# moskewcz/boda

Hardware: AMD Instinct MI355X
Metric: effective TFLOP/s (2*M*N*K / time), whole job (higher is better)
Workload: dtype f32

## Files before the change

__graft_entry__.py:

```python
from __future__ import annotations
import os
import sys

ROOT = os.path.dirname(os.path.abspath(__file__))
if ROOT not in sys.path:
    sys.path.insert(0, ROOT)


def build() -> None:
    from boda_amd import build as b
    so = b.build()
    assert os.path.exists(so)
    import boda_amd.rtc as rtc
    from boda_amd import gen_data
    from boda_amd.op import read_ops
    assert rtc._lib.bodahip_abi_version() == 1
    rtc.compile_offline(gen_data.SRC, use_cache=True)
    n = 0
    gold = os.path.join(ROOT, "tests", "golden", "ops")
    for fn in ("sgemm-ops-full.txt", "sgemm-ops-debug-half.txt", "conv-ops-1-5-20-nin-alex-gn.txt", "conv-ops-debug.txt", "conv-ops-debug-tmp.txt",
               "bck-conv-ops.txt", "bck-ops.txt", "bck-pipe-ops.txt", "bck-fuse-ops.txt", "bck-graph-ops.txt", "bck-shards-ops.txt", "resnet-ops.txt", "fwd-deps-ops.txt", "sgd-ops.txt", "bn-ops.txt", "bconv-fb-ops.txt", "bconv-bf16-ops.txt"):
        if not os.path.exists(os.path.join(gold, fn)):
            continue
        for op in read_ops(os.path.join(gold, fn)):
            rtc.prebuild(op); n += 1
    import bench
    from boda_amd.cnn_op import OpTune, add_codegen_annotations
    from boda_amd import conv_pipe
    rtc.compile_offline(conv_pipe.FWD_SRC, use_cache=True)
    for op in bench.alexnet_b256_ops() + bench.nin_ops() + bench.net_conv_ops("googlenet_conv", 64) + bench.net_conv_ops("resnet-50", 64):
        rtc.prebuild(op); n += 1
    for op in bench.net_conv_ops("googlenet_conv", 2) + bench.net_conv_ops("resnet-50", 2) + bench.alexnet_b256_ops(2) + bench.nin_ops(3):
        rtc.prebuild(op); n += 1
    for op in bench.alexnet_b256_ops() + bench.nin_ops() + bench.sgemm_full_ops() + bench.net_conv_ops("googlenet_conv", 64) + bench.net_conv_ops("resnet-50", 64):
        rtc.prebuild(add_codegen_annotations(op, OpTune(hip_dtype="bf16"))); n += 1
    from boda_amd import nhwc
    rtc.compile_offline(nhwc.XPOSE_SRC, use_cache=True)
    for op in bench.net_conv_ops("googlenet_conv", 64) + bench.net_conv_ops("resnet-50", 64) + bench.net_conv_ops("googlenet_conv", 2) + bench.net_conv_ops("resnet-50", 2):
        for out in ("", "f32"):
            rtc.prebuild(add_codegen_annotations(op, OpTune(hip_dtype="bf16", hip_layout="nhwc", hip_out=out))); n += 1
    for net in ("googlenet_conv", "resnet-50"):
        for out in ("", "f32"):
            el = [x for x in (add_codegen_annotations(op, OpTune(hip_dtype="bf16", hip_layout="nhwc", hip_out=out)) for op in bench.net_conv_ops(net, 64)) if nhwc.multi_eligible(x)]
            m = nhwc.annotate_multi(el); rtc.prebuild(m); n += 1
            for t in ("64x128x64x2x2x2", "128x128x64x2x2x2", "32x128x64x1x4x2", "32x128x64x1x4x2x1x32x2", "128x64x32x2x2x2x1x32x4", "64x64x32x2x2x2x1x32x3"):
                rtc.prebuild(m, tile=t); n += 1
    from boda_amd.conv_pipe import ConvPipeFwd, DryRtc
    seen = set()
    resnet_small = lambda batch: conv_pipe.resnet50(batch, 64)
    for make, batches, kw in ((conv_pipe.googlenet_conv, (64, 1, 3), {}), (conv_pipe.nin_imagenet, (256, 128, 2), {}), (conv_pipe.alexnet_ng_conv, (256, 2), {}),
                              (conv_pipe.resnet50, (64,), {}), (conv_pipe.resnet50, (64,), {"fuse_residual": False}), (resnet_small, (2,), {}), (resnet_small, (2,), {"fuse_residual": False})):
        for batch in batches:
            dry = DryRtc(); ConvPipeFwd(dry, OpTune(hip_dtype="bf16", hip_layout="nhwc"), **kw).init(make(batch))
            for fi in dry.infos:
                if fi.op is not None and fi.op.has_func_name() and fi.op.get_func_name().startswith("hip_conv_nhwc") and "_xpose_" not in fi.op.get_func_name() and fi.op.to_str() not in seen:
                    seen.add(fi.op.to_str()); rtc.prebuild(fi.op); n += 1
    for batch in (256, 128):
        dry = DryRtc(); ConvPipeFwd(dry).init(conv_pipe.nin_imagenet(batch))
        for fi in dry.infos:
            if fi.op is not None and fi.op.has_func_name() and fi.op.get_func_name() == "hip_conv_k1_chain" and fi.op.to_str() not in seen:
                seen.add(fi.op.to_str()); rtc.prebuild(fi.op); n += 1
    dry = DryRtc(); ConvPipeFwd(dry).init(resnet_small(2))
    for fi in dry.infos:
        if fi.op is not None and fi.op.has_func_name() and fi.op.get_func_name() in ("hip_conv", "hip_chan_affine", "hip_reduce", "hip_zero_if_non_pos") and fi.op.to_str() not in seen:
            seen.add(fi.op.to_str()); rtc.prebuild(fi.op); n += 1
    _recompile_with_the_wheels_hiprtc()
    b.build_adapter()
    from oracle import boda_oracle, ref_cucl
    boda_oracle.build()
    n_ref = ref_cucl.build()
    print(f"oracle/_ref/cucl: {n_ref} reference kernels compiled" if n_ref else "oracle/_ref/cucl: no Boda checkout here, prebuilt files (if any) left alone")
    print(f"build ok: {so}; {n} ops pre-specialised into {os.path.join(ROOT, 'boda_amd', '_kcache')}")


def _fp32_conv_ops():
    import bench
    ops = bench.alexnet_b256_ops() + bench.nin_ops() + bench.nin_ops(128) + bench.net_conv_ops("googlenet_conv", 64) + bench.net_conv_ops("resnet-50", 64)
    return ops + bench.net_conv_ops("googlenet_conv", 2) + bench.net_conv_ops("resnet-50", 2) + bench.alexnet_b256_ops(2) + bench.nin_ops(3)


def _recompile_with_the_wheels_hiprtc() -> None:
    import subprocess
    code = ("import torch, os, sys; sys.path.insert(0, %r); os.environ['BODAHIP_CACHE_REFRESH'] = 'bodahip_conv_big'\n"
            "import __graft_entry__ as g, boda_amd.rtc as rtc\n"
            "n = 0\n"
            "for op in g._fp32_conv_ops():\n"
            "    if rtc.explain_plan(op).startswith('bodahip_conv_big_f32'): rtc.prebuild(op); n += 1\n"
            "print(n)" % ROOT)
    r = subprocess.run([sys.executable, "-c", code], capture_output=True, text=True, timeout=1800)
    if r.returncode != 0:
        print("build: second pass (the wheel's hiprtc for the staging-wave convolution kernels) skipped: " + (r.stderr.strip().splitlines() or ["?"])[-1])
    else:
        print(f"build: {r.stdout.strip().splitlines()[-1]} staging-wave convolution plans recompiled by the PyTorch wheel's hiprtc")


def smoke() -> None:
    import numpy as np
    from boda_amd.cnn_op import OpTune, add_codegen_annotations
    from boda_amd.op import parse_op
    from boda_amd.ops_prof import OpsBackend, profile_rcg_call
    from boda_amd.rtc import make_rtc
    from oracle import boda_oracle as bo
    rtc = make_rtc("(be=hip)", 0)
    rtc.init()
    be = OpsBackend(rtc)
    sg = parse_op("(str_vals=(type=sgemm),nda_vals=(a=(dims=(K=192,M=256)),b=(dims=(K=192,N=320)),c=(dims=(M=256,N=320))))")
    outs, prc = profile_rcg_call(be, add_codegen_annotations(sg, OpTune()), 5, include_ins=True)
    assert np.array_equal(outs["c"], bo.sgemm(outs["a"], outs["b"])), "smoke: sgemm mismatch vs oracle"
    cv = parse_op("(str_vals=(type=Convolution),nda_vals=(biases=(dims=(out_chan=64)),filts=(dims=(out_chan=64,in_chan=32,y=5,x=5)),"
                  "in=(dims=(img=5,chan=32,y=14,x=14)),in_pad=(tn=none,dims=(y=2,x=2)),kern_sz=(tn=none,dims=(y=5,x=5)),"
                  "out=(dims=(img=5,chan=64,y=14,x=14)),out_chans=(tn=uint32_t,v=64),stride=(tn=none,dims=(y=1,x=1))))")
    outs, prc2 = profile_rcg_call(be, add_codegen_annotations(cv, OpTune()), 5, include_ins=True)
    want = bo.conv_fwd(outs["in"], outs["filts"], outs["biases"], (1, 1), (2, 2), True)
    assert np.array_equal(outs["out"], want), "smoke: conv mismatch vs oracle"
    t_s, t_c = "64x64x16x2x2x4x1x32x2x3", "64x128x16x2x2x2x1x32x2x2"
    outs, prc3 = profile_rcg_call(be, add_codegen_annotations(sg, OpTune(hip_tile=t_s)), 5, include_ins=True, tile=t_s)
    assert prc3.launch["kernel"] == "bodahip_sgemm_big_f32" and np.array_equal(outs["c"], bo.sgemm(outs["a"], outs["b"])), "smoke: staging-wave sgemm mismatch vs oracle"
    outs, prc4 = profile_rcg_call(be, add_codegen_annotations(cv, OpTune(hip_tile=t_c)), 5, include_ins=True, tile=t_c)
    assert prc4.launch["kernel"] == "bodahip_conv_big_f32" and np.array_equal(outs["out"], want), "smoke: staging-wave conv mismatch vs oracle"
    print(f"smoke ok on {rtc.get_plat_tag()}: sgemm {prc.rt_secs*1e6:.1f} us [{prc.launch['cfg']}] / [{prc3.launch['cfg']}], conv {prc2.rt_secs*1e6:.1f} us [{prc2.launch['cfg']}] / [{prc4.launch['cfg']}]")
    rtc.close()


if __name__ == "__main__":
    build()
    if len(sys.argv) > 1 and sys.argv[1] == "smoke":
        smoke()
```

boda_amd/csrc/kernels/sgemm_big_f32.hip:

```cpp

#ifndef __HIPCC_RTC__
#include <hip/hip_runtime.h>
#endif

typedef float f32x16 __attribute__((ext_vector_type(16)));
typedef float f32x4 __attribute__((ext_vector_type(4)));
typedef unsigned u32x2 __attribute__((ext_vector_type(2)));
#ifndef GROUP_I
#define GROUP_I 8
#endif
#ifndef BKS
#define BKS 8
#endif
#ifndef PF
#define PF 2
#endif
#ifndef TBI
#define TBI 256
#endif
#ifndef TBJ
#define TBJ 256
#endif
#ifndef WI
#define WI 2
#endif
#ifndef WJ
#define WJ 4
#endif
#ifndef MINW
#define MINW 1
#endif
#ifndef MULPRIO
#define MULPRIO 1
#endif
#ifndef STGPRIO
#define STGPRIO 0
#endif
#ifndef NSTG
#define NSTG 4
#endif

struct gemm_args_t {
  float const *I; float const *J; float *D; float const *bias;
  int Mi, Nj, K;
  int ldI, ldJ, ldD;
  int C, H, W, OH, OW;
  int tiles_i, tiles_j;
  int splitk, kt_per;
  float *ws; long ws_slab;
  unsigned I_bytes, J_bytes;
  unsigned D_bytes;
  int out_ctot, out_coff;
  int const *ktab; int ktab_n;
  long bsI, bsJ, bsD;
};

namespace {
constexpr int kNMW = WI * WJ;
static_assert(kNMW == 8 || kNMW == 4, "eight (or four) multiplying waves");
constexpr int kTI = TBI / (WI * 32), kTJ = TBJ / (WJ * 32);
static_assert(TBI % (WI * 32) == 0 && TBJ % (WJ * 32) == 0 && (kTI == 4 || kTI == 2 || kTI == 1) && (kTJ == 2 || kTJ == 1), "wave tile: 4 | 2 | 1 row blocks x 2 | 1 column blocks");
constexpr int kLDI = TBI + 4, kLDJ = TBJ + 4;
constexpr int kImgI = BKS * kLDI, kImgJ = BKS * kLDJ, kImg2 = kImgI + kImgJ;
constexpr int kNLI = BKS * (TBI / 4) / 256, kNLJ = BKS * (TBJ / 4) / 256;
static_assert((BKS * (TBI / 4)) % 256 == 0 && (BKS * (TBJ / 4)) % 256 == 0, "whole float4 units per staging thread");
constexpr int kKK = BKS / 2;
constexpr int kU = (NSTG == 3) ? 3 * PF : ((PF > NSTG) ? PF : NSTG);
constexpr int kD = NSTG - 1;
static_assert(NSTG == 3 || NSTG == 4, "NSTG: 3 | 4");
constexpr int kOOB = (int)0x80000000;
static_assert(BKS % 4 == 0 && (PF == 2 || PF == 4), "BKS % 4 == 0, PF: 2 | 4");
typedef __amdgpu_buffer_rsrc_t rsrc_t;
__device__ __forceinline__ rsrc_t make_rsrc(float const *p, unsigned bytes) { return __builtin_amdgcn_make_buffer_rsrc((void *)p, 0, (int)bytes, 0x00020000); }
__device__ __forceinline__ f32x4 bload4(rsrc_t r, int voff, int soff) { return __builtin_bit_cast(f32x4, __builtin_amdgcn_raw_buffer_load_b128(r, voff, soff, 0)); }
}

#if (TBI / (WI * 32)) == 4
typedef f32x4 avec_t;
#elif (TBI / (WI * 32)) == 2
typedef float2 avec_t;
#else
typedef float avec_t;
#endif
#if (TBJ / (WJ * 32)) == 2
typedef float2 bvec_t;
#else
typedef float bvec_t;
#endif
namespace {
__device__ __forceinline__ float vget(f32x4 const &v, int i) { return v[i]; }
__device__ __forceinline__ float vget(float2 const &v, int i) { return i ? v.y : v.x; }
__device__ __forceinline__ float vget(float const &v, int) { return v; }
}

extern "C" __global__ __launch_bounds__((kNMW + 4) * 64, MINW) void KNAME(gemm_args_t const p) {
  __shared__ __attribute__((aligned(16))) float sm[NSTG * kImg2];
  int const lane = threadIdx.x & 63;
  int const wave = __builtin_amdgcn_readfirstlane(threadIdx.x >> 6);
  bool const stager = wave >= kNMW;

  int tile_i, tile_j;
  {
    int const bid = blockIdx.x, nb = p.tiles_i * p.tiles_j;
    int const q = nb >> 3, rr = nb & 7, xcd = bid & 7, idx = bid >> 3;
    int const nid = ((xcd < rr) ? xcd * (q + 1) : rr * (q + 1) + (xcd - rr) * q) + idx;
    int const group_sz = GROUP_I * p.tiles_j, gid = nid / group_sz, first_i = gid * GROUP_I;
    int const gsz = min(p.tiles_i - first_i, GROUP_I), in_g = nid - gid * group_sz;
    tile_i = first_i + in_g % gsz; tile_j = in_g / gsz;
  }
  int const i0 = tile_i * TBI, j0 = tile_j * TBJ;
  int const nkt = (p.K + BKS - 1) / BKS;
  int const nkt_pad = (nkt + kU - 1) / kU * kU;

  if (stager) {
#if STGPRIO
    __builtin_amdgcn_s_setprio(STGPRIO);
#endif
    int const tid = threadIdx.x - kNMW * 64;
    rsrc_t const rI = make_rsrc(p.I, p.I_bytes), rJ = make_rsrc(p.J, p.J_bytes);
    int goffI[kNLI], goffJ[kNLJ], loffI[kNLI], loffJ[kNLJ], krowI[kNLI], krowJ[kNLJ];
#pragma unroll
    for (int n = 0; n < kNLI; ++n) {
      int const c = tid + n * 256, kr = c / (TBI / 4), x = 4 * (c % (TBI / 4));
      krowI[n] = kr; loffI[n] = kr * kLDI + x;
      goffI[n] = (i0 + x < p.Mi) ? ((kr * p.ldI + i0 + x) * 4) : kOOB;
    }
#pragma unroll
    for (int n = 0; n < kNLJ; ++n) {
      int const c = tid + n * 256, kr = c / (TBJ / 4), x = 4 * (c % (TBJ / 4));
      krowJ[n] = kr; loffJ[n] = kImgI + kr * kLDJ + x;
      goffJ[n] = (j0 + x < p.Nj) ? ((kr * p.ldJ + j0 + x) * 4) : kOOB;
    }
    auto gloadI = [&](int n, int kt) -> f32x4 { return bload4(rI, (kt * BKS + krowI[n] < p.K) ? goffI[n] : kOOB, min(kt, nkt - 1) * (BKS * 4) * p.ldI); };
    auto gloadJ = [&](int n, int kt) -> f32x4 { return bload4(rJ, (kt * BKS + krowJ[n] < p.K) ? goffJ[n] : kOOB, min(kt, nkt - 1) * (BKS * 4) * p.ldJ); };
    auto lstoreI = [&](int n, int stage, f32x4 const &v) { *reinterpret_cast<f32x4 *>(sm + stage * kImg2 + loffI[n]) = v; };
    auto lstoreJ = [&](int n, int stage, f32x4 const &v) { *reinterpret_cast<f32x4 *>(sm + stage * kImg2 + loffJ[n]) = v; };
    f32x4 ringI[PF][kNLI], ringJ[PF][kNLJ];
#pragma unroll
    for (int u = 0; u < PF; ++u) {
#pragma unroll
      for (int n = 0; n < kNLI; ++n) ringI[u][n] = gloadI(n, u);
#pragma unroll
      for (int n = 0; n < kNLJ; ++n) ringJ[u][n] = gloadJ(n, u);
    }
#pragma unroll
    for (int t = 0; t < kD; ++t) {
#pragma unroll
      for (int n = 0; n < kNLI; ++n) { lstoreI(n, t, ringI[t % PF][n]); ringI[t % PF][n] = gloadI(n, t + PF); }
#pragma unroll
      for (int n = 0; n < kNLJ; ++n) { lstoreJ(n, t, ringJ[t % PF][n]); ringJ[t % PF][n] = gloadJ(n, t + PF); }
    }
    asm volatile("s_waitcnt lgkmcnt(0)\n s_barrier" ::: "memory");
    for (int kb = 0; kb < nkt_pad; kb += kU) {
#pragma unroll
      for (int u = 0; u < kU; ++u) {
#pragma unroll
        for (int n = 0; n < kNLI; ++n) { lstoreI(n, (u + kD) % NSTG, ringI[(u + kD) % PF][n]); ringI[(u + kD) % PF][n] = gloadI(n, kb + u + kD + PF); }
#pragma unroll
        for (int n = 0; n < kNLJ; ++n) { lstoreJ(n, (u + kD) % NSTG, ringJ[(u + kD) % PF][n]); ringJ[(u + kD) % PF][n] = gloadJ(n, kb + u + kD + PF); }
        asm volatile("s_waitcnt lgkmcnt(%0)\n s_barrier" :: "n"(kNLI + kNLJ) : "memory");
      }
    }
    return;
  }

#if MULPRIO
  __builtin_amdgcn_s_setprio(MULPRIO);
#endif
  int const wi = wave / WJ, wj = wave % WJ;
  float const *const a_base = sm + (lane >> 5) * kLDI + wi * (kTI * 32) + kTI * (lane & 31);
  float const *const b_base = sm + kImgI + (lane >> 5) * kLDJ + wj * (kTJ * 32) + kTJ * (lane & 31);
  f32x16 acc[kTI][kTJ];
#pragma unroll
  for (int t = 0; t < kTI; ++t)
#pragma unroll
    for (int u = 0; u < kTJ; ++u)
#pragma unroll
      for (int r = 0; r < 16; ++r) acc[t][u][r] = 0.f;

  asm volatile("s_barrier" ::: "memory");
  avec_t a[2]; bvec_t b[2];
  a[0] = *reinterpret_cast<avec_t const *>(a_base); b[0] = *reinterpret_cast<bvec_t const *>(b_base);
  static_assert(kKK % 2 == 0, "an even number of k pairs per step (the operand double buffer carries over from step to step)");
  for (int kb = 0; kb < nkt_pad; kb += kU) {
#pragma unroll
    for (int s = 0; s < kU; ++s) {
      float const *const A = a_base + (s % NSTG) * kImg2, *const B = b_base + (s % NSTG) * kImg2;
      float const *const An = a_base + ((s + 1) % NSTG) * kImg2, *const Bn = b_base + ((s + 1) % NSTG) * kImg2;
#pragma unroll
      for (int kk = 0; kk < kKK; ++kk) {
        if (kk + 1 < kKK) { a[(kk + 1) & 1] = *reinterpret_cast<avec_t const *>(A + (kk + 1) * 2 * kLDI); b[(kk + 1) & 1] = *reinterpret_cast<bvec_t const *>(B + (kk + 1) * 2 * kLDJ); }
#if NSTG == 4
        else { a[0] = *reinterpret_cast<avec_t const *>(An); b[0] = *reinterpret_cast<bvec_t const *>(Bn); }
#endif
        __builtin_amdgcn_sched_barrier(0);
        avec_t const ca = a[kk & 1]; bvec_t const cb = b[kk & 1];
#pragma unroll
        for (int t = 0; t < kTI; ++t)
#pragma unroll
          for (int u = 0; u < kTJ; ++u) acc[t][u] = __builtin_amdgcn_mfma_f32_32x32x2f32(vget(ca, t), vget(cb, u), acc[t][u], 0, 0, 0);
        __builtin_amdgcn_sched_barrier(0);
      }
#if NSTG == 4
      asm volatile("s_barrier" ::: "memory");
#else
      asm volatile("s_waitcnt lgkmcnt(0)\n s_barrier" ::: "memory");
      a[0] = *reinterpret_cast<avec_t const *>(An); b[0] = *reinterpret_cast<bvec_t const *>(Bn);
#endif
    }
  }

  {
    rsrc_t const rD = make_rsrc(p.D, p.D_bytes);
    int const j = j0 + wj * (kTJ * 32) + kTJ * (lane & 31);
    int const il = i0 + wi * (kTI * 32) + kTI * 4 * (lane >> 5);
// ... 17 lines not shown
```

boda_amd/csrc/native_plan.cc:

```cpp
#include "native_internal.h"

namespace bodahip {

bool parse_tile(string const &s, tile_cfg_t &c) {
  int v[11] = {0, 0, 0, 0, 0, 0, 0, 0, 0, 0, 0}; int n = 0; string cur;
  for (size_t i = 0; i <= s.size(); ++i) {
    if (i == s.size() || s[i] == 'x' || s[i] == ':') { if (cur.empty() || n >= 11) return false; v[n++] = atoi(cur.c_str()); cur.clear(); }
    else if (s[i] >= '0' && s[i] <= '9') cur.push_back(s[i]); else return false;
  }
  if (n < 5) return false;
  c.BI = v[0]; c.BJ = v[1]; c.BK = v[2]; c.WI = v[3]; c.WJ = v[4]; c.MINW = (n >= 6) ? v[5] : 1; c.SPLITK = (n >= 7) ? v[6] : 1; c.MT = (n >= 8) ? v[7] : 32; c.PF = (n >= 9) ? v[8] : 1; c.SW = (n >= 10) ? v[9] : 0; c.KHO = (n >= 11) ? v[10] : 0;
  return true;
}
static void check_cfg(tile_cfg_t const &c, bool gather, bool patch = false) {
  int const nt = c.WI * c.WJ * 64;
  bool ok = c.BI > 0 && c.BJ > 0 && c.BK > 0 && c.WI > 0 && c.WJ > 0 && nt <= 1024 && c.threads() <= 1024 && (c.MT == 32 || c.MT == 16) && (c.BI % (c.WI * c.MT) == 0) && (c.BJ % (c.WJ * c.MT) == 0) &&
            (c.BK % 2 == 0) && (c.MT == 32 || c.BK % 4 == 0) && (c.BI % 4 == 0) && (c.BJ % 4 == 0);
  if (gather) ok = ok && ((c.BK * c.BJ) % nt == 0);
  if (gather) ok = ok && (nt % c.BJ == 0) && (c.BJ % 64 == 0);
  ok = ok && c.SPLITK >= 1 && c.SPLITK <= 64 && c.MINW >= 1 && (c.PF == 1 || c.PF == 2 || c.PF == 4 || c.PF == 6 || c.PF == 8);
  ok = ok && c.KHO >= 0 && c.KHO <= 64 && (c.KHO <= 1 || (c.SPLITK == 1 && c.SW == 0));
  if (c.PF > 2) ok = ok && ((long)c.PF * c.BK * (c.BI + c.BJ) / nt <= 192);
  int const accs = (c.BI / (c.WI * c.MT)) * (c.BJ / (c.WJ * c.MT));
  ok = ok && accs * (c.MT == 32 ? 16 : 4) <= 256;
// ... 96 lines not shown
  } else {
    if (g.C <= 64 && g.OC > 128 && g.OC <= 512 && g.OC % 256 == 0 && Nj >= 150000) { WI = 8; WJ = 1; OCB = g.OC / 256; CB = 2; }
    else return false;
    if (regs(OCB, CB) > 250 || lds(WI, OCB) > 80 * 1024) return false;
  }
  if (!MINW) { int const r = regs(OCB, CB); MINW = std::max(1, std::min(8, 512 / r)); int const wpw = (WI * WJ + 3) / 4;
               long const by_lds = std::max(1l, (160l * 1024) / lds(WI, OCB)); MINW = (int)std::max(1l, std::min((long)MINW, by_lds * wpw)); }
  p.stream = true; p.kname = "bodahip_k1_stream_f32";
  p.cfg.BI = WI * OCB * 32; p.cfg.BJ = WJ * CB * 32; p.cfg.BK = g.C; p.cfg.WI = WI; p.cfg.WJ = WJ; p.cfg.MINW = MINW; p.cfg.SPLITK = 1; p.cfg.MT = 32; p.cfg.PF = 1;
  p.defs = {"-DKC=" + std::to_string(g.C), "-DHW=" + std::to_string(g.OH * g.OW), "-DWI=" + std::to_string(WI), "-DWJ=" + std::to_string(WJ),
            "-DOCB=" + std::to_string(OCB), "-DCB=" + std::to_string(CB), "-DMINW=" + std::to_string(MINW), string("-DRELU=") + (g.relu ? "1" : "0"),
            string("-DEDGE_OC=") + ((g.OC % (WI * OCB * 32)) ? "1" : "0")};
  if (char const *e = getenv("BODAHIP_EXTRA_DEFS")) { std::istringstream is(e); string tok; while (is >> tok) p.defs.push_back(tok); }
  return true;
}

static void bf16_cfg(tile_cfg_t &c, bool gather, long Mi = 0, long Nj = 0, long K = 0, int num_cus = 0, bool explicit_tile = false) {
  if (c.MT != 32) { c.MT = 32; c.BI = 64; c.BJ = 64; c.WI = 2; c.WJ = 2; }
  if (c.BK != 32 && c.BK != 64) c.BK = 32;
  c.PF = 1;
  if (!explicit_tile) {
    c.SPLITK = 1;
    if (Mi > 0 && num_cus > 0 && getenv("BODAHIP_NO_BF16_SPLITK") == nullptr) {
      long const nkt = (K + c.BK - 1) / c.BK;
      long const tiles = ((Mi + c.BI - 1) / c.BI) * ((Nj + c.BJ - 1) / c.BJ), tiles128 = ((Mi + 127) / 128) * ((Nj + 127) / 128);
      if (tiles <= num_cus && nkt >= 64) {
        long s = std::min<long>(16, (2l * num_cus + tiles128 - 1) / tiles128);
        s = std::min<long>(s, nkt / 8);
        if (s >= 2) { c.BI = 128; c.BJ = 128; c.WI = 2; c.WJ = 2; c.MINW = 2; c.SPLITK = (int)s; }
      }
    }
  }
  int const nt = c.threads();
  bool ok = (c.BI % (c.WI * 32) == 0) && (c.BJ % (c.WJ * 32) == 0) && ((c.BI * c.BK / 8) % nt == 0) && ((c.BJ * c.BK / 8) % nt == 0) && nt <= 1024 &&
            (c.BI / (c.WI * 32)) * (c.BJ / (c.WJ * 32)) * 16 <= 256 && 4ull * (c.BK + 8) * (c.BI + c.BJ) <= 160 * 1024;
  if (gather) ok = ok && (c.BJ % 64 == 0) && (nt % c.BJ == 0);
  if (!ok) unsup_err("native bf16 kernel: unsupported tile configuration " + c.str());
}

static char const *const kStg64 = "64x64x16x2x2x4x1x32x2x3";
plan_t plan_sgemm(uint32_t M, uint32_t N, uint32_t K, int num_cus, string const &tile, bool bf16, int batch, bool allow_big) {
  plan_t p; p.kname = bf16 ? "bodahip_sgemm_bf16" : "bodahip_sgemm_f32"; p.bf16 = bf16;
  p.cfg = choose_cfg((int)M, (int)std::min<uint64_t>((uint64_t)N * batch, 0x7fffffffull), (int)K, num_cus, false, bf16);
  if (!tile.empty()) { if (!parse_tile(tile, p.cfg)) rt_err("bad sgemm_tile '" + tile + "'"); }
  if (bf16) {
    bf16_cfg(p.cfg, false, M, N, K, num_cus, !tile.empty());
    p.defs = cfg_defs(p.cfg); p.defs.push_back("-DI_MODE=0"); p.defs.push_back("-DJ_MODE=0"); p.defs.push_back("-DEPI=0");
    if (p.cfg.SPLITK > 1) p.defs.push_back("-DSPLITK=1");
    return p;
  }
  if (!tile.empty() && p.cfg.SW == 3) {
    tile_cfg_t const &c = p.cfg;
    int const nmw = c.WI * c.WJ, ti = (c.WI > 0 && c.BI % (c.WI * 32) == 0) ? c.BI / (c.WI * 32) : 0, tj = (c.WJ > 0 && c.BJ % (c.WJ * 32) == 0) ? c.BJ / (c.WJ * 32) : 0;
    bool const ok = (nmw == 8 || nmw == 4) && (ti == 4 || ti == 2 || ti == 1) && (tj == 2 || tj == 1) && c.BK >= 4 && c.BK <= 32 && c.BK % 4 == 0 && (c.BK * (c.BI / 4)) % 256 == 0 &&
                    (c.BK * (c.BJ / 4)) % 256 == 0 && (c.PF == 2 || c.PF == 4) && c.MT == 32 && c.SPLITK == 1 && c.MINW >= 1 && c.MINW <= 8 && 4l * 4 * c.BK * (c.BI + c.BJ + 8) <= 160 * 1024;
    if (!ok || batch != 1 || M % 4 || N % 4 || !allow_big) unsup_err("hip_sgemm: unsupported staging-wave tile " + c.str() + " (8 | 4 multiplying waves of 4 | 2 | 1 x 2 | 1 blocks, whole float4 units per staging thread, M and N multiples of 4)");
    p.big = true; p.kname = "bodahip_sgemm_big_f32"; p.cfg.KHO = 0;
    p.defs = {"-DBKS=" + std::to_string(c.BK), "-DPF=" + std::to_string(c.PF), "-DTBI=" + std::to_string(c.BI), "-DTBJ=" + std::to_string(c.BJ), "-DWI=" + std::to_string(c.WI),
              "-DWJ=" + std::to_string(c.WJ), "-DMINW=" + std::to_string(c.MINW)};
    if (char const *x = getenv("BODAHIP_EXTRA_DEFS")) { std::istringstream is(x); string tok; while (is >> tok) p.defs.push_back(tok); }
    return p;
  }
  bool const big_tile = (p.cfg.BI == 256 || p.cfg.BI == 128) && (p.cfg.BJ == 256 || p.cfg.BJ == 128);
  bool const want_big = big_tile && ((p.cfg.WI == 3 && p.cfg.WJ == 4) || (p.cfg.BI == 256 && p.cfg.BJ == 256));
  if (allow_big && batch == 1 && want_big && p.cfg.MT == 32 && p.cfg.SPLITK == 1 && M % 4 == 0 && N % 4 == 0) {
    char const *e = getenv("BODAHIP_SGEMM_BIG");
    if (!(e && string(e) == "off")) {
      int bks = 8, pf = 4;
      if (!tile.empty() && p.cfg.WI == 3 && p.cfg.BK >= 4 && p.cfg.BK <= 32 && p.cfg.BK % 4 == 0) bks = p.cfg.BK;
      if (e && *e) { if (sscanf(e, "%dx%d", &bks, &pf) != 2 || bks < 4 || bks > 32 || bks % 4 || (pf != 2 && pf != 4)) rt_err(string("bad BODAHIP_SGEMM_BIG '") + e + "' (off | BKSxPF)"); }
      if (bks * (p.cfg.BI / 4) % 256 || bks * (p.cfg.BJ / 4) % 256) bks = 8;
      int const minw = (p.cfg.BI == 128 && p.cfg.BJ == 128) ? ((!tile.empty() && p.cfg.MINW >= 1) ? std::min(p.cfg.MINW, 2) : 2) : 1;
      p.big = true; p.kname = "bodahip_sgemm_big_f32"; p.cfg.BK = bks; p.cfg.PF = pf; p.cfg.WI = 3; p.cfg.WJ = 4; p.cfg.MINW = minw;
      p.defs = {"-DBKS=" + std::to_string(bks), "-DPF=" + std::to_string(pf)};
      if (!(p.cfg.BI == 256 && p.cfg.BJ == 256)) {
        bool const tall = (p.cfg.BI == 256 && p.cfg.BJ == 128);
        p.defs.push_back("-DTBI=" + std::to_string(p.cfg.BI)); p.defs.push_back("-DTBJ=" + std::to_string(p.cfg.BJ));
        p.defs.push_back(string("-DWI=") + (tall ? "4" : "2")); p.defs.push_back(string("-DWJ=") + (tall ? "2" : "4")); p.defs.push_back("-DMINW=" + std::to_string(minw));
      }
      if (char const *x = getenv("BODAHIP_EXTRA_DEFS")) { std::istringstream is(x); string tok; while (is >> tok) p.defs.push_back(tok); }
      return p;
    }
  }
  if (tile.empty() && allow_big && batch == 1 && p.cfg.BI == 64 && p.cfg.BJ == 64 && p.cfg.MT == 32 && p.cfg.SPLITK == 1 && M % 4 == 0 && N % 4 == 0 && K >= 512 && getenv("BODAHIP_NO_SGEMM_STG64") == nullptr) {
    char const *e = getenv("BODAHIP_SGEMM_BIG");
    if (!(e && string(e) == "off")) return plan_sgemm(M, N, K, num_cus, kStg64, false, 1, true);
  }
  p.cfg.KHO = 0;
  check_cfg(p.cfg, false);
  p.defs = cfg_defs(p.cfg);
  p.defs.push_back(string("-DI_MODE=") + ((M % 4 == 0) ? "0" : "1"));
  p.defs.push_back(string("-DJ_MODE=") + ((N % 4 == 0) ? "0" : "1"));
  p.defs.push_back("-DEPI=0");
  if (p.cfg.SPLITK > 1) p.defs.push_back("-DSPLITK=1");
  return p;
}
bool plan_patch_bf16(conv_geom_t const &g, int num_cus, plan_t &p) {
  if (getenv("BODAHIP_NO_PATCH16")) return false;
  int const taps = g.KH * g.KW;
  if (!(g.SX == 1 && taps >= 2 && g.KH >= g.SY && g.C % 8 == 0 && g.C >= 16)) return false;
  if (g.OH == 1 && g.OW == 1 && g.PY == 0 && g.PX == 0 && g.KH == g.H && g.KW == g.W) return false;
  int cg = 1; while (cg * taps < 16) ++cg;
  if (char const *e = getenv("BODAHIP_PATCH16_CG")) { if (atoi(e) > 0) cg = atoi(e); }
  if (cg > 8) return false;
  int const np = cg * taps + ((cg * taps) & 1);
  long const Nj = (long)g.B * g.OH * g.OW;
  int const wp = g.W + 2 * g.PX;
  auto lds = [&](int bi, int bj) {
    int const rows_max = (bj - 2) / g.OW + 2, seg_max0 = (g.OH - 1 + rows_max - 1) / g.OH + 1, seg_max = std::min(seg_max0, rows_max);
    long const cs = (long)((rows_max - seg_max) * g.SY + seg_max * g.KH) * wp;
    return 16l * ((long)np * bi + cg * cs);
  };
// ... 550 lines not shown
      long const R = (ti1 * tj_all) / num_cus; if (R < 1) continue;
      long const tj1 = std::min(tj_all - 1, (R * num_cus) / ti1); if (tj1 < 1) continue;
      long const n1 = tj1 * m.bj; if (n1 >= Nj) continue;
      double const t_main = (double)((ti1 * tj1 + num_cus - 1) / num_cus) * m.bi * m.bj / m.base;
      for (cand_t const &t : cands) {
        tile_cfg_t c2; c2.BI = t.bi; c2.BJ = t.bj; c2.BK = 16; c2.WI = t.wi; c2.WJ = t.wj; c2.MINW = 2; c2.SPLITK = 1; c2.MT = 32; c2.PF = 2; c2.SW = 2; c2.KHO = 0;
        conv_big_form_t f2; if (!conv_big_form(g, c2, f2) || f2.jmode != (patchy ? 7 : 5)) continue;
        long tt = 0; double const tsum = t_main + t_of(t, Nj - n1, tt);
        if (tsum < t_best) { t_best = tsum; best_n1 = n1; m_best = &m; t_best_c = &t; }
      }
    }
    if (m_best) {
      tile_cfg_t c1; c1.BI = m_best->bi; c1.BJ = m_best->bj; c1.BK = 16; c1.WI = m_best->wi; c1.WJ = m_best->wj; c1.MINW = 2; c1.SPLITK = 1; c1.MT = 32; c1.PF = 2; c1.SW = 2; c1.KHO = 0;
      tile_cfg_t c2 = c1; c2.BI = t_best_c->bi; c2.BJ = t_best_c->bj; c2.WI = t_best_c->wi; c2.WJ = t_best_c->wj;
      bp = plan_conv_big(g, c1); plan_t const tp = plan_conv_big(g, c2);
      bp.split_pels = best_n1; bp.tail_cfg = tp.cfg; bp.tail_defs = tp.defs;
    }
  }
  return bp;
}


static double launch_model(long n, double a, int s, double r, int cus) {
  long const per = (long)cus * s, full = n / per, rest = n - full * per;
  double t = (double)full * s * a / r;
  if (rest) { long const k = (rest + cus - 1) / cus; double const eff = (k >= s) ? 1.0 : 0.6 + 0.4 * (double)(k - 1) / (double)(s - 1); t += (double)k * a / (r * eff); }
  return t;
}
static char const *const kTail64 = getenv("BODAHIP_SGEMM_TAIL64") ? getenv("BODAHIP_SGEMM_TAIL64") : ((getenv("BODAHIP_SGEMM_BIG") && string(getenv("BODAHIP_SGEMM_BIG")) == "off") || getenv("BODAHIP_NO_SGEMM_STG64")) ? "64x64x32x2x2x2x1x32x2" : kStg64;
sgemm_split_t plan_sgemm_split(uint32_t M, uint32_t N, uint32_t K, int num_cus) {
  sgemm_split_t sp;
  if (getenv("BODAHIP_NO_SGEMM_SPLIT") || M % 4 || N % 4 || K < 512 || M < 1024 || N < 1024) return sp;
  long const ti = (M + 255) / 256, tj = (N + 255) / 256;
  if (ti * tj < num_cus) return sp;
  double const r_big = getenv("BODAHIP_SGEMM_RBIG") ? atof(getenv("BODAHIP_SGEMM_RBIG")) : 1.04, r_mid = 1.0, r_small = 0.93;
  auto small_n = [&](uint32_t rows, int b) { return (long)((rows + b - 1) / b) * (long)((N + b - 1) / b); };
  sp.t_single = std::min(launch_model(ti * tj, 1.0, 1, r_big, num_cus), launch_model(small_n(M, 128), 0.25, 2, r_mid, num_cus));
  double best = sp.t_single * 0.975;
  for (long R = 1; R < ti; ++R) {
    uint32_t const m_main = (uint32_t)(R * 256), rows = M - m_main;
    double const tm = launch_model(R * tj, 1.0, 1, r_big, num_cus);
    double const t128 = tm + launch_model(small_n(rows, 128), 0.25, 2, r_mid, num_cus) + 0.004;
    double const t64 = tm + launch_model(small_n(rows, 64), 0.0625, 2, r_small, num_cus) + 0.004;
    char const *const force = getenv("BODAHIP_SGEMM_SPLIT_TAIL");
    if (force && atoi(force) == 128) { if (t128 < best) { best = t128; sp.m_main = m_main; sp.tail_tile = "128x128x16x2x2x2"; } continue; }
    if (force && atoi(force) == 64) { if (t64 < best) { best = t64; sp.m_main = m_main; sp.tail_tile = kTail64; } continue; }
    if (t128 < best) { best = t128; sp.m_main = m_main; sp.tail_tile = "128x128x16x2x2x2"; }
    if (t64 < best) { best = t64; sp.m_main = m_main; sp.tail_tile = kTail64; }
  }
  sp.t_split = best;
  return sp;
}

string sgemm_wide_tile(uint32_t M, uint32_t N, uint32_t K, long cus) {
  if (M % 4 || N % 4 || K < 512 || getenv("BODAHIP_NO_SGEMM_256X128")) return string();
  if (char const *e = getenv("BODAHIP_SGEMM_BIG")) { if (string(e) == "off") return string(); }
  long const t256 = (long)((M + 255) / 256) * ((N + 255) / 256), t128 = (long)((M + 255) / 256) * ((N + 127) / 128);
  double const eff = (double)t128 / (double)(((t128 + cus - 1) / cus) * cus);
  return (t256 >= cus && eff >= 0.95) ? string("256x128x8x3x4x1") : string();
}

bool parse_parts_env(uint32_t M, uint32_t N, uint32_t K, std::vector<sgemm_part_t> &out) {
  char const *e = getenv("BODAHIP_SGEMM_PARTS"); if (!e || M != N || N != K) return false;
  string const v = e, key = std::to_string(M) + ":"; size_t const at = (";" + v).find(";" + key); if (at == string::npos) return false;
  size_t const b = at + key.size(), en = v.find(';', b); string const spec = v.substr(b, en == string::npos ? string::npos : en - b);
  std::istringstream is(spec); string one;
  while (std::getline(is, one, '/')) {
    sgemm_part_t q; char tl[128];
    if (sscanf(one.c_str(), "%u,%u,%u,%u,%127s", &q.m0, &q.rows, &q.n0, &q.cols, tl) != 5) rt_err("bad BODAHIP_SGEMM_PARTS entry '" + one + "'");
    q.tile = tl; out.push_back(q);
  }
  uint64_t area = 0; for (auto const &q : out) { if (q.m0 % 4 || q.n0 % 4 || q.m0 + q.rows > M || q.n0 + q.cols > N || !q.rows || !q.cols) rt_err("bad BODAHIP_SGEMM_PARTS rectangle"); area += (uint64_t)q.rows * q.cols; }
  if (area != (uint64_t)M * N) rt_err("BODAHIP_SGEMM_PARTS: the rectangles do not add up to c");
  return true;
}

struct sgemm_form_t { char const *tile; int bi, bj, s; double r, lone; };
static sgemm_form_t const kFormQ = {"256x256x16x2x4x1x1x32x2", 256, 256, 1, 1.0, 1.0}, kFormW = {"256x128x8x3x4x1", 256, 128, 2, 1.0127, 0.82}, kFormS = {kStg64, 64, 64, 4, 0.913, 0.5};
static double form_cost(sgemm_form_t const &f, uint32_t rows, uint32_t cols, int cus) {
  long const n = (long)((rows + f.bi - 1) / f.bi) * ((cols + f.bj - 1) / f.bj), per = (long)cus * f.s;
  double const a = (double)f.bi * f.bj / 65536.0, round = f.s * a / f.r;
  if (n <= per) { long const k = (n + cus - 1) / cus; double const eff = (f.s == 1 || k >= f.s) ? 1.0 : f.lone + (1.0 - f.lone) * (double)(k - 1) / (double)(f.s - 1);
                  return (double)k * a / (f.r * eff); }
  if (f.s >= 4) return (double)n / (double)per * round;
  return (double)((n + per - 1) / per) * round;
}
struct sgemm_parts_plan_t { std::vector<sgemm_part_t> parts; double t = 1e30; };
static sgemm_parts_plan_t plan_parts_rec(uint32_t m0, uint32_t rows, uint32_t n0, uint32_t cols, int cus, double ovh, int depth) {
  sgemm_parts_plan_t best;
  for (sgemm_form_t const *f : {&kFormQ, &kFormW, &kFormS}) {
    double const t = form_cost(*f, rows, cols, cus) + ovh;
    if (t < best.t) { best.t = t; sgemm_part_t q; q.m0 = m0; q.rows = rows; q.n0 = n0; q.cols = cols; q.tile = f->tile; best.parts = {q}; }
  }
  if (depth <= 0) return best;
  for (sgemm_form_t const *f : {&kFormQ, &kFormW}) {
    long const per = (long)cus * f->s, tj = (cols + f->bj - 1) / f->bj, ti = (rows + f->bi - 1) / f->bi;
    for (long R = 1; R < ti; ++R) {
      if ((R * tj) % per) continue;
      uint32_t const r1 = (uint32_t)(R * f->bi);
      sgemm_parts_plan_t rest = plan_parts_rec(m0 + r1, rows - r1, n0, cols, cus, ovh, depth - 1);
      double const t = form_cost(*f, r1, cols, cus) + ovh + rest.t;
      if (t < best.t) { best.t = t; sgemm_part_t q; q.m0 = m0; q.rows = r1; q.n0 = n0; q.cols = cols; q.tile = f->tile; best.parts = {q}; best.parts.insert(best.parts.end(), rest.parts.begin(), rest.parts.end()); }
    }
    for (long C = 1; C < tj; ++C) {
      if ((C * ti) % per) continue;
      uint32_t const c1 = (uint32_t)(C * f->bj);
      sgemm_parts_plan_t rest = plan_parts_rec(m0, rows, n0 + c1, cols - c1, cus, ovh, depth - 1);
      double const t = form_cost(*f, rows, c1, cus) + ovh + rest.t;
      if (t < best.t) { best.t = t; sgemm_part_t q; q.m0 = m0; q.rows = rows; q.n0 = n0; q.cols = c1; q.tile = f->tile; best.parts = {q}; best.parts.insert(best.parts.end(), rest.parts.begin(), rest.parts.end()); }
    }
  }
  return best;
}
std::vector<sgemm_part_t> plan_sgemm_parts(uint32_t M, uint32_t N, uint32_t K, int cus) {
  std::vector<sgemm_part_t> none;
  if (getenv("BODAHIP_NO_SGEMM_PARTS") || getenv("BODAHIP_NO_SGEMM_SPLIT") || M % 4 || N % 4 || K < 512 || M < 1024 || N < 1024 || (long)((M + 255) / 256) * ((N + 255) / 256) < cus) return none;
  if (char const *e = getenv("BODAHIP_SGEMM_BIG")) { if (string(e) == "off") return none; }
  if (M % 64 || N % 64) return none;
  double const ovh = 25.7 / (double)K;
  sgemm_parts_plan_t pp = plan_parts_rec(0, M, 0, N, cus, ovh, 3);
  for (uint32_t R = 1024; R < M; R += 1024) {
    sgemm_parts_plan_t const t1 = plan_parts_rec(0, R, 0, N, cus, ovh, 2), t2 = plan_parts_rec(R, M - R, 0, N, cus, ovh, 2);
    if (t1.t + t2.t < pp.t) { pp.t = t1.t + t2.t; pp.parts = t1.parts; pp.parts.insert(pp.parts.end(), t2.parts.begin(), t2.parts.end()); }
  }
  for (uint32_t C = 1024; C < N; C += 1024) {
    sgemm_parts_plan_t const t1 = plan_parts_rec(0, M, 0, C, cus, ovh, 2), t2 = plan_parts_rec(0, M, C, N - C, cus, ovh, 2);
    if (t1.t + t2.t < pp.t) { pp.t = t1.t + t2.t; pp.parts = t1.parts; pp.parts.insert(pp.parts.end(), t2.parts.begin(), t2.parts.end()); }
  }
  if (pp.parts.size() < 2) return none;
  double t_now = std::min(form_cost(kFormQ, M, N, cus), form_cost(kFormW, M, N, cus)) + ovh;
  sgemm_split_t const sp = plan_sgemm_split(M, N, K, cus);
  if (sp.m_main && sgemm_wide_tile(M, N, K, cus).empty()) t_now = std::min(t_now, form_cost(kFormQ, sp.m_main, N, cus) + form_cost(kFormS, M - sp.m_main, N, cus) + 2 * ovh);
  return (pp.t < 0.98 * t_now) ? pp.parts : none;
}



static void check_bconv_cfg(tile_cfg_t const &c, bool filts) {
  int const nt = c.WI * c.WJ * 64;
// ... 286 lines not shown
```

Before: 144.5.

## Add twelve-wave 256x192 staging-wave sgemm tile with peeled ring loop

Adds a 4x3 (or 3x4) twelve-multiplying-wave configuration of the staging-wave sgemm kernel with a 256x192 block tile and a configurable stage count of 3. The wide-tile chooser can now pick it when its cost model beats the 256x128 form and the wave-count efficiency holds. The staging loop is split into a main part that uses raw buffer loads with computed offsets and a tail part that keeps the bounds-handled loads, with scheduling barriers between phases. The aim is better data reuse per block and less address overhead in the steady state. The cost is a 1024-thread block with more register and LDS pressure, plus reliance on an estimated cost ratio.

```diff
diff --git a/__graft_entry__.py b/__graft_entry__.py
--- a/__graft_entry__.py
+++ b/__graft_entry__.py
@@ -19,7 +19,7 @@
     n = 0
     gold = os.path.join(ROOT, "tests", "golden", "ops")
     for fn in ("sgemm-ops-full.txt", "sgemm-ops-debug-half.txt", "conv-ops-1-5-20-nin-alex-gn.txt", "conv-ops-debug.txt", "conv-ops-debug-tmp.txt",
-               "bck-conv-ops.txt", "bck-ops.txt", "bck-pipe-ops.txt", "bck-fuse-ops.txt", "bck-graph-ops.txt", "bck-shards-ops.txt", "resnet-ops.txt", "fwd-deps-ops.txt", "sgd-ops.txt", "bn-ops.txt", "bconv-fb-ops.txt", "bconv-bf16-ops.txt"):
+               "bck-conv-ops.txt", "bck-ops.txt", "bck-pipe-ops.txt", "bck-fuse-ops.txt", "bck-graph-ops.txt", "bck-shards-ops.txt", "resnet-ops.txt", "fwd-deps-ops.txt", "sgd-ops.txt", "bn-ops.txt", "bconv-fb-ops.txt", "bconv-bf16-ops.txt", "sgemm-w12-ops.txt"):
         if not os.path.exists(os.path.join(gold, fn)):
             continue
         for op in read_ops(os.path.join(gold, fn)):
@@ -116,9 +116,12 @@
     t_s, t_c = "64x64x16x2x2x4x1x32x2x3", "64x128x16x2x2x2x1x32x2x2"
     outs, prc3 = profile_rcg_call(be, add_codegen_annotations(sg, OpTune(hip_tile=t_s)), 5, include_ins=True, tile=t_s)
     assert prc3.launch["kernel"] == "bodahip_sgemm_big_f32" and np.array_equal(outs["c"], bo.sgemm(outs["a"], outs["b"])), "smoke: staging-wave sgemm mismatch vs oracle"
+    t_w = "256x192x16x4x3x4x1x32x2x3"
+    outs, prc5 = profile_rcg_call(be, add_codegen_annotations(sg, OpTune(hip_tile=t_w)), 5, include_ins=True, tile=t_w)
+    assert prc5.launch["kernel"] == "bodahip_sgemm_big_f32" and prc5.launch["block"] == 1024 and np.array_equal(outs["c"], bo.sgemm(outs["a"], outs["b"])), "smoke: twelve-wave sgemm mismatch vs oracle"
     outs, prc4 = profile_rcg_call(be, add_codegen_annotations(cv, OpTune(hip_tile=t_c)), 5, include_ins=True, tile=t_c)
     assert prc4.launch["kernel"] == "bodahip_conv_big_f32" and np.array_equal(outs["out"], want), "smoke: staging-wave conv mismatch vs oracle"
-    print(f"smoke ok on {rtc.get_plat_tag()}: sgemm {prc.rt_secs*1e6:.1f} us [{prc.launch['cfg']}] / [{prc3.launch['cfg']}], conv {prc2.rt_secs*1e6:.1f} us [{prc2.launch['cfg']}] / [{prc4.launch['cfg']}]")
+    print(f"smoke ok on {rtc.get_plat_tag()}: sgemm {prc.rt_secs*1e6:.1f} us [{prc.launch['cfg']}] / [{prc3.launch['cfg']}] / [{prc5.launch['cfg']}], conv {prc2.rt_secs*1e6:.1f} us [{prc2.launch['cfg']}] / [{prc4.launch['cfg']}]")
     rtc.close()
 
 
diff --git a/boda_amd/csrc/kernels/sgemm_big_f32.hip b/boda_amd/csrc/kernels/sgemm_big_f32.hip
--- a/boda_amd/csrc/kernels/sgemm_big_f32.hip
+++ b/boda_amd/csrc/kernels/sgemm_big_f32.hip
@@ -35,6 +35,9 @@
 #endif
 #ifndef STGPRIO
 #define STGPRIO 0
+#endif
+#ifndef STGRING
+#define STGRING 1
 #endif
 #ifndef NSTG
 #define NSTG 4
@@ -57,7 +60,7 @@
 
 namespace {
 constexpr int kNMW = WI * WJ;
-static_assert(kNMW == 8 || kNMW == 4, "eight (or four) multiplying waves");
+static_assert(kNMW == 12 || kNMW == 8 || kNMW == 4, "twelve, eight or four multiplying waves");
 constexpr int kTI = TBI / (WI * 32), kTJ = TBJ / (WJ * 32);
 static_assert(TBI % (WI * 32) == 0 && TBJ % (WJ * 32) == 0 && (kTI == 4 || kTI == 2 || kTI == 1) && (kTJ == 2 || kTJ == 1), "wave tile: 4 | 2 | 1 row blocks x 2 | 1 column blocks");
 constexpr int kLDI = TBI + 4, kLDJ = TBJ + 4;
@@ -73,6 +76,7 @@
 typedef __amdgpu_buffer_rsrc_t rsrc_t;
 __device__ __forceinline__ rsrc_t make_rsrc(float const *p, unsigned bytes) { return __builtin_amdgcn_make_buffer_rsrc((void *)p, 0, (int)bytes, 0x00020000); }
 __device__ __forceinline__ f32x4 bload4(rsrc_t r, int voff, int soff) { return __builtin_bit_cast(f32x4, __builtin_amdgcn_raw_buffer_load_b128(r, voff, soff, 0)); }
+template <bool B> struct bool_c { static constexpr bool value = B; };
 }
 
 #if (TBI / (WI * 32)) == 4
@@ -151,6 +155,33 @@
       for (int n = 0; n < kNLJ; ++n) { lstoreJ(n, t, ringJ[t % PF][n]); ringJ[t % PF][n] = gloadJ(n, t + PF); }
     }
     asm volatile("s_waitcnt lgkmcnt(0)\n s_barrier" ::: "memory");
+#if STGRING
+    int const nfull = p.K / BKS;
+    auto step = [&](auto tail, int u, int kb) __attribute__((always_inline)) {
+      int const slot = (u + kD) % PF, stage = (u + kD) % NSTG, kt = kb + u + kD + PF;
+#pragma unroll
+      for (int n = 0; n < kNLI; ++n) lstoreI(n, stage, ringI[slot][n]);
+#pragma unroll
+      for (int n = 0; n < kNLJ; ++n) lstoreJ(n, stage, ringJ[slot][n]);
+      __builtin_amdgcn_sched_barrier(0);
+#pragma unroll
+      for (int n = 0; n < kNLI; ++n) ringI[slot][n] = decltype(tail)::value ? gloadI(n, kt) : bload4(rI, goffI[n], kt * (BKS * 4) * p.ldI);
+#pragma unroll
+      for (int n = 0; n < kNLJ; ++n) ringJ[slot][n] = decltype(tail)::value ? gloadJ(n, kt) : bload4(rJ, goffJ[n], kt * (BKS * 4) * p.ldJ);
+      __builtin_amdgcn_sched_barrier(0);
+      asm volatile("s_waitcnt lgkmcnt(%0)\n s_barrier" :: "n"(kNLI + kNLJ) : "memory");
+      __builtin_amdgcn_sched_barrier(0);
+    };
+    int kb = 0;
+    for (; kb + kU + kD + PF <= nfull; kb += kU) {
+#pragma unroll
+      for (int u = 0; u < kU; ++u) step(bool_c<false>(), u, kb);
+    }
+    for (; kb < nkt_pad; kb += kU) {
+#pragma unroll
+      for (int u = 0; u < kU; ++u) step(bool_c<true>(), u, kb);
+    }
+#else
     for (int kb = 0; kb < nkt_pad; kb += kU) {
 #pragma unroll
       for (int u = 0; u < kU; ++u) {
@@ -161,6 +192,7 @@
         asm volatile("s_waitcnt lgkmcnt(%0)\n s_barrier" :: "n"(kNLI + kNLJ) : "memory");
       }
     }
+#endif
     return;
   }
 
diff --git a/boda_amd/csrc/native_plan.cc b/boda_amd/csrc/native_plan.cc
--- a/boda_amd/csrc/native_plan.cc
+++ b/boda_amd/csrc/native_plan.cc
@@ -172,12 +172,16 @@
   if (!tile.empty() && p.cfg.SW == 3) {
     tile_cfg_t const &c = p.cfg;
     int const nmw = c.WI * c.WJ, ti = (c.WI > 0 && c.BI % (c.WI * 32) == 0) ? c.BI / (c.WI * 32) : 0, tj = (c.WJ > 0 && c.BJ % (c.WJ * 32) == 0) ? c.BJ / (c.WJ * 32) : 0;
-    bool const ok = (nmw == 8 || nmw == 4) && (ti == 4 || ti == 2 || ti == 1) && (tj == 2 || tj == 1) && c.BK >= 4 && c.BK <= 32 && c.BK % 4 == 0 && (c.BK * (c.BI / 4)) % 256 == 0 &&
-                    (c.BK * (c.BJ / 4)) % 256 == 0 && (c.PF == 2 || c.PF == 4) && c.MT == 32 && c.SPLITK == 1 && c.MINW >= 1 && c.MINW <= 8 && 4l * 4 * c.BK * (c.BI + c.BJ + 8) <= 160 * 1024;
-    if (!ok || batch != 1 || M % 4 || N % 4 || !allow_big) unsup_err("hip_sgemm: unsupported staging-wave tile " + c.str() + " (8 | 4 multiplying waves of 4 | 2 | 1 x 2 | 1 blocks, whole float4 units per staging thread, M and N multiples of 4)");
-    p.big = true; p.kname = "bodahip_sgemm_big_f32"; p.cfg.KHO = 0;
+    int const nstg = c.KHO ? c.KHO : 4;
+    bool const w12 = (nmw == 12) && ((c.WI == 4 && c.WJ == 3) || (c.WI == 3 && c.WJ == 4)) && ti == 2 && tj == 2 && c.MINW <= 4;
+    bool const ok = (nmw == 8 || nmw == 4 || w12) && (ti == 4 || ti == 2 || ti == 1) && (tj == 2 || tj == 1) && c.BK >= 4 && c.BK <= 32 && c.BK % 4 == 0 && (c.BK * (c.BI / 4)) % 256 == 0 &&
+                    (c.BK * (c.BJ / 4)) % 256 == 0 && (c.PF == 2 || c.PF == 4) && c.MT == 32 && c.SPLITK == 1 && c.MINW >= 1 && c.MINW <= 8 && (nstg == 3 || nstg == 4) && 4l * nstg * c.BK * (c.BI + c.BJ + 8) <= 160 * 1024;
+    if (!ok || batch != 1 || M % 4 || N % 4 || !allow_big) unsup_err("hip_sgemm: unsupported staging-wave tile " + c.str() + " (8 | 4 multiplying waves of 4 | 2 | 1 x 2 | 1 blocks or 4 x 3 | 3 x 4 of 2 x 2, whole float4 units per staging thread, M and N multiples of 4)");
+    p.big = true; p.kname = "bodahip_sgemm_big_f32";
     p.defs = {"-DBKS=" + std::to_string(c.BK), "-DPF=" + std::to_string(c.PF), "-DTBI=" + std::to_string(c.BI), "-DTBJ=" + std::to_string(c.BJ), "-DWI=" + std::to_string(c.WI),
               "-DWJ=" + std::to_string(c.WJ), "-DMINW=" + std::to_string(c.MINW)};
+    if (c.KHO) p.defs.push_back("-DNSTG=" + std::to_string(nstg));
+    p.cfg.KHO = 0;
     if (char const *x = getenv("BODAHIP_EXTRA_DEFS")) { std::istringstream is(x); string tok; while (is >> tok) p.defs.push_back(tok); }
     return p;
   }
@@ -834,14 +838,6 @@
   return sp;
 }
 
-string sgemm_wide_tile(uint32_t M, uint32_t N, uint32_t K, long cus) {
-  if (M % 4 || N % 4 || K < 512 || getenv("BODAHIP_NO_SGEMM_256X128")) return string();
-  if (char const *e = getenv("BODAHIP_SGEMM_BIG")) { if (string(e) == "off") return string(); }
-  long const t256 = (long)((M + 255) / 256) * ((N + 255) / 256), t128 = (long)((M + 255) / 256) * ((N + 127) / 128);
-  double const eff = (double)t128 / (double)(((t128 + cus - 1) / cus) * cus);
-  return (t256 >= cus && eff >= 0.95) ? string("256x128x8x3x4x1") : string();
-}
-
 bool parse_parts_env(uint32_t M, uint32_t N, uint32_t K, std::vector<sgemm_part_t> &out) {
   char const *e = getenv("BODAHIP_SGEMM_PARTS"); if (!e || M != N || N != K) return false;
   string const v = e, key = std::to_string(M) + ":"; size_t const at = (";" + v).find(";" + key); if (at == string::npos) return false;
@@ -859,6 +855,7 @@
 
 struct sgemm_form_t { char const *tile; int bi, bj, s; double r, lone; };
 static sgemm_form_t const kFormQ = {"256x256x16x2x4x1x1x32x2", 256, 256, 1, 1.0, 1.0}, kFormW = {"256x128x8x3x4x1", 256, 128, 2, 1.0127, 0.82}, kFormS = {kStg64, 64, 64, 4, 0.913, 0.5};
+static sgemm_form_t const kFormT = {"256x192x16x4x3x4x1x32x2x3", 256, 192, 1, getenv("BODAHIP_SGEMM_RW12") ? atof(getenv("BODAHIP_SGEMM_RW12")) : 0.963, 1.0};
 static double form_cost(sgemm_form_t const &f, uint32_t rows, uint32_t cols, int cus) {
   long const n = (long)((rows + f.bi - 1) / f.bi) * ((cols + f.bj - 1) / f.bj), per = (long)cus * f.s;
   double const a = (double)f.bi * f.bj / 65536.0, round = f.s * a / f.r;
@@ -867,6 +864,18 @@
   if (f.s >= 4) return (double)n / (double)per * round;
   return (double)((n + per - 1) / per) * round;
 }
+string sgemm_wide_tile(uint32_t M, uint32_t N, uint32_t K, long cus) {
+  if (M % 4 || N % 4 || K < 512 || getenv("BODAHIP_NO_SGEMM_256X128")) return string();
+  if (char const *e = getenv("BODAHIP_SGEMM_BIG")) { if (string(e) == "off") return string(); }
+  long const t256 = (long)((M + 255) / 256) * ((N + 255) / 256), t128 = (long)((M + 255) / 256) * ((N + 127) / 128);
+  double const eff = (double)t128 / (double)(((t128 + cus - 1) / cus) * cus);
+  if (!(t256 >= cus && eff >= 0.95)) return string();
+  long const t192 = (long)((M + 255) / 256) * ((N + 191) / 192);
+  double const eff192 = (double)t192 / (double)(((t192 + cus - 1) / cus) * cus);
+  if (!getenv("BODAHIP_NO_SGEMM_W12") && eff192 >= 0.95 && form_cost(kFormT, M, N, (int)cus) < form_cost(kFormW, M, N, (int)cus)) return string(kFormT.tile);
+  return string(kFormW.tile);
+}
+
 struct sgemm_parts_plan_t { std::vector<sgemm_part_t> parts; double t = 1e30; };
 static sgemm_parts_plan_t plan_parts_rec(uint32_t m0, uint32_t rows, uint32_t n0, uint32_t cols, int cus, double ovh, int depth) {
   sgemm_parts_plan_t best;
```

New measurement: 149.9, median of 6. 3.7% higher.
